# facebookresearch/PoseDiffusion

Measured on AMD Instinct MI355X. Metric: sequences/sec (20-frame, GGS on), higher is better.
Workload: dtype f32 (GGS, attention, LayerNorm, DDPM update, every accumulation); the encoder GEMMs multiply fp16 hi + lo operand pairs (22 bits, static power-of-two scales) with fp32 accumulation -- `exact_mode` is the same pipe with them on the exact-fp32 matrix instruction

## Files before the change

include/pd_engine.h:

```cpp
#ifndef PD_ENGINE_H
#define PD_ENGINE_H

#include <stdint.h>

#ifdef __cplusplus
extern "C" {
#endif

#define PD_OK 0
#define PD_ERR_INVALID_ARG (-1)
#define PD_ERR_UNSUPPORTED (-2)
#define PD_ERR_HIP (-3)
#define PD_ERR_STATE (-4)

#define PD_MAX_LAYERS 16
#define PD_POSE_DIM 9

typedef struct pd_engine pd_engine;

typedef struct pd_layer_weights {
    const float *norm1_w, *norm1_b;
    const float *in_proj_w, *in_proj_b;
    const float *out_proj_w, *out_proj_b;
    const float *norm2_w, *norm2_b;
// ... 88 lines not shown
                                 const double *kp2, const int64_t *i12, int n_frames, int height, int width,
                                 const pd_match_hints *hints, void *stream);


int pd_ggs_guide(pd_engine *eng, float *model_mean, int B, int N, int t, const pd_ggs_cfg *cfg,
                 float *stats_out, void *stream);

int pd_ggs_stage_iters(const pd_ggs_cfg *cfg, int *iters_out5);

int pd_ggs_optimize(pd_engine *eng, float *model_mean, int B, int N, int update_R, int update_T,
                    int update_FL, const pd_ggs_cfg *cfg, float *stats_out, float *trace_out,
                    void *stream);

int pd_ggs_loss_grad(pd_engine *eng, const float *x, int B, int N, int update_R, int update_T,
                     int update_FL, const pd_ggs_cfg *cfg, float *loss_out, float *grad_out,
                     void *stream);


#define PD_OPT_DENOISER_SPLIT 2
#define PD_OPT_DENOISER_FUSED_ATTN 5
#define PD_OPT_DENOISER_LONG_ATTN 6
#define PD_OPT_GGS_MAX_FRAMES 7
#define PD_OPT_GGS_LONG_PAIR_ITEMS 8
int pd_engine_set_option(pd_engine *eng, int option, int value);
#define PD_OPT_WEIGHTS_NON_FINITE 4
int pd_engine_get_option(pd_engine *eng, int option, int *value_out);

int pd_sample(pd_engine *eng, const float *z, const float *noise, int B, int N, int cond_start_step,
              const pd_ggs_cfg *ggs, float *pose_out, float *process_out, float *stats_out,
              int use_graph, void *stream);

#define PD_PHASE_ALL 0
#define PD_PHASE_UNGUIDED 1
#define PD_PHASE_GUIDED 2
int pd_sample_phase(pd_engine *eng, const float *z, const float *noise, int B, int N, int cond_start_step,
                    const pd_ggs_cfg *ggs, int phase, float *pose_out, float *process_out, float *stats_out,
                    int use_graph, void *stream);

int pd_pose_to_camera(pd_engine *eng, const float *enc, int n_cameras, float *R_out, float *T_out,
                      float *focal_out, void *stream);
int pd_pose_to_camera_ex(pd_engine *eng, const float *enc, int n_cameras, float *R_out, float *T_out,
                         float *focal_out, float log_focal_length_bias, float min_focal_length, float max_focal_length,
                         void *stream);

int pd_camera_to_pose(const float *R, const float *T, const float *focal, int n, float log_focal_length_bias,
                      float min_focal_length, float max_focal_length, float *enc_out, void *stream);
// ... 58 lines not shown
```

posediffusion_amd/_lib.py:

```python
from __future__ import annotations

import ctypes as C
import os
import subprocess

_HERE = os.path.dirname(os.path.abspath(__file__))
LIB_PATH = os.environ.get("PD_ENGINE_LIB") or os.path.join(_HERE, "lib", "libpd_engine.so")
CSRC_DIR = os.path.join(_HERE, "csrc")
HEADER_PATH = os.path.normpath(os.path.join(_HERE, "..", "include", "pd_engine.h"))

PD_MAX_LAYERS = 16

c_float_p = C.POINTER(C.c_float)


class pd_layer_weights(C.Structure):
    _fields_ = [(n, C.c_void_p) for n in (
        "norm1_w", "norm1_b", "in_proj_w", "in_proj_b", "out_proj_w", "out_proj_b",
        "norm2_w", "norm2_b", "linear1_w", "linear1_b", "linear2_w", "linear2_b")]


class pd_weights(C.Structure):
    _fields_ = (
        [(n, C.c_int32) for n in ("d_model", "nhead", "dim_ff", "num_layers", "z_dim", "n_harmonic",
# ... 27 lines not shown
class pd_vit_weights(C.Structure):
    _fields_ = ([(n, C.c_int32) for n in ("dim", "depth", "num_heads", "mlp_hidden", "patch_size", "pos_grid", "reserved0", "reserved1")]
                + [(n, C.c_void_p) for n in ("patch_w", "patch_b", "cls_token", "pos_embed", "norm_w", "norm_b")]
                + [("layers", pd_vit_layer_weights * 16)])


PD_GGS_CFG_FORCE_ONE_HOP = 1
PD_GGS_CFG_NO_LDS_STAGING = 2
PD_GGS_CFG_WAVES8 = 4
PD_WEIGHTS_PRED_X0 = 1
PD_WEIGHTS_POST_NORM = 2
PD_WEIGHTS_NO_PIVOT = 4
PD_WEIGHTS_GENERIC = 8
PD_GGS_CFG_LANE_ITEMS = 8
PD_GGS_CFG_NO_LANE_ITEMS = 16
PD_GGS_CFG_XCHG_SPREAD = 32
PD_GGS_CFG_LONG_FRAMES = 64
PD_OPT_DENOISER_SPLIT = 2
PD_OPT_WEIGHTS_NON_FINITE = 4
PD_OPT_DENOISER_FUSED_ATTN = 5
PD_OPT_DENOISER_LONG_ATTN = 6
PD_OPT_GGS_MAX_FRAMES = 7
PD_OPT_GGS_LONG_PAIR_ITEMS = 8
PD_DROP_ATTN, PD_DROP_RESID1, PD_DROP_FF, PD_DROP_RESID2, PD_DROP_ALL = 1, 2, 4, 8, 15
PD_TR_OPT_MAX_FRAMES, PD_TR_OPT_LONG_ATTN = 1, 2
PD_MATCH_HINT_ONE_ORDER = 1 << 30


class pd_ggs_cfg(C.Structure):
    _fields_ = [("alpha", C.c_float), ("learning_rate", C.c_float), ("iter_num", C.c_int32),
                ("sampson_max", C.c_float), ("min_matches", C.c_int32), ("momentum", C.c_float),
                ("wgs_per_seq", C.c_int32), ("reserved", C.c_int32)]


class pd_match_hints(C.Structure):
    _fields_ = [("max_pairs", C.c_int32), ("max_matches_per_pair", C.c_int32)]


_vp, _i, _i64 = C.c_void_p, C.c_int, C.c_int64
SIGNATURES = {
    "pd_engine_create": (_i, [C.POINTER(pd_weights), _i, _i, C.POINTER(_vp)]),
    "pd_engine_destroy": (None, [_vp]),
    "pd_last_error": (C.c_char_p, []),
    "pd_version": (C.c_char_p, []),
    "pd_denoise_step": (_i, [_vp, _vp, _vp, _i, _i, _i, _vp, _vp]),
    "pd_engine_set_q_tables": (_i, [_vp, _vp, _vp]),
# ... 96 lines not shown
```

posediffusion_amd/csrc/pd_engine.hip:

```cpp
#include "pd_internal.h"

#include <algorithm>

#include <math.h>
#include <stdarg.h>
#include <string.h>

static thread_local char g_err[1024] = "";

void pd_set_error(const char *fmt, ...) {
    va_list ap;
    va_start(ap, fmt);
    vsnprintf(g_err, sizeof(g_err), fmt, ap);
    va_end(ap);
}

extern "C" const char *pd_last_error(void) { return g_err; }
extern "C" const char *pd_version(void) { return "pd_engine 0.1 gfx950"; }

__global__ void pd_finish_kernel(const float *__restrict__ mean, const float *__restrict__ noise, float sigma, int n,
                                 float *__restrict__ out, const int *__restrict__ nf, int n_frames) {
    const int i = blockIdx.x * blockDim.x + threadIdx.x;
    if (i >= n) return;
    if (nf) {
// ... 693 lines not shown
            unsigned long long *fresh = nullptr;
            if (hipMalloc((void **)&fresh, sizeof(unsigned long long) * 2 * granules * eng->max_B) != hipSuccess) {
                (void)hipGetLastError();
                pd_set_error("pd_engine_set_option: PD_OPT_GGS_MAX_FRAMES = %d: hipMalloc of %zu B for the exchange region failed; the limit stays %d",
                             value, sizeof(unsigned long long) * 2 * granules * eng->max_B, eng->ggs_max_frames);
                return PD_ERR_HIP;
            }
            (void)hipFree(eng->d_xchg);
            eng->d_xchg = fresh;
            eng->xchg_granules = granules;
        }
        for (auto &g : eng->graphs) (void)hipGraphExecDestroy(g.second);
        eng->graphs.clear();
        eng->ggs_max_frames = value;
        break;
    }
    case PD_OPT_GGS_LONG_PAIR_ITEMS:
        if (value < 0 || value > 1) {
            pd_set_error("pd_engine_set_option: PD_OPT_GGS_LONG_PAIR_ITEMS takes 0 or 1 (got %d)", value);
            return PD_ERR_INVALID_ARG;
        }
        eng->ggs_long_pair_items = value;
        break;
    case 3:
        if (value == 0) break;
        pd_set_error("pd_engine_set_option: option 3 (the persistent small-batch denoiser launch of round 3) is no longer built: it measured "
                     "2.4 x slower than the multi-launch path (profiles/round3_small_persistent.txt; source parked under tools/parked/)");
        return PD_ERR_UNSUPPORTED;
    default:
        pd_set_error("pd_engine_set_option: unknown option %d", option);
        return PD_ERR_INVALID_ARG;
    }
    return PD_OK;
}

extern "C" int pd_engine_get_option(pd_engine *eng, int option, int *value_out) {
    if (!eng || !value_out) {
        pd_set_error("pd_engine_get_option: NULL argument");
        return PD_ERR_INVALID_ARG;
    }
    switch (option) {
    case PD_OPT_DENOISER_SPLIT: *value_out = eng->den_split; break;
    case PD_OPT_DENOISER_FUSED_ATTN: *value_out = eng->den_fused_attn; break;
    case PD_OPT_DENOISER_LONG_ATTN: *value_out = eng->den_long_attn; break;
    case PD_OPT_GGS_MAX_FRAMES: *value_out = eng->ggs_max_frames; break;
    case PD_OPT_GGS_LONG_PAIR_ITEMS: *value_out = eng->ggs_long_pair_items; break;
    case PD_OPT_WEIGHTS_NON_FINITE: *value_out = pd_denoiser_weights_non_finite(eng) ? 1 : 0; break;
    default:
        pd_set_error("pd_engine_get_option: unknown option %d", option);
        return PD_ERR_INVALID_ARG;
    }
    return PD_OK;
}

extern "C" int pd_time_kernel(pd_engine *eng, int what, int B, int N, const pd_ggs_cfg *cfg, int reps, float *ms_out,
                              void *stream) {
    if (!eng || !ms_out || reps <= 0 || B <= 0 || B > eng->max_B || N <= 0 || N > eng->max_N) {
        pd_set_error("pd_time_kernel: invalid arguments");
        return PD_ERR_INVALID_ARG;
    }
    if (what != 0) {
        PD_TRY(check_cfg(cfg, "pd_time_kernel"));
        PD_TRY(pd_ggs_frames_unsupported(eng, N, "pd_time_kernel"));
    }
    hipStream_t s = (hipStream_t)stream;
    struct CountsOff {
        pd_engine *e;
        int B;
        explicit CountsOff(pd_engine *e_) : e(e_), B(e_->nf_B) { e->nf_B = 0; }
// ... 112 lines not shown
```

posediffusion_amd/csrc/pd_ggs.hip:

```cpp
#include "pd_internal.h"

#include <algorithm>
#include <math.h>
#include <stdlib.h>
#include <string.h>

#pragma clang fp contract(on)

#ifndef PD_GGS_PROF12
#define PD_GGS_PROF12 0
#endif
#ifndef PD_GGS_ABLATE
#define PD_GGS_ABLATE 0
#endif

#ifndef PD_GGS_MIN_WAVES_PER_SIMD
#define PD_GGS_MIN_WAVES_PER_SIMD 2
#endif

#include "pd_ggs_lds.h"
#include "pd_ggs_dev.h"
#include "pd_ggs_sampson.h"
#include "pd_ggs_kernels.h"
#include "pd_ggs_lane.inc"
// ... 46 lines not shown
    max_items = 0;
    for (int b = 0; b < B; ++b) {
        const PdSeqDesc &d = eng->seqs[b].desc;
        if (d.M <= 0 || !eng->seqs[b].blob) {
            pd_set_error("pd_ggs: sequence slot %d has no matches (call pd_ggs_set_matches)", b);
            return PD_ERR_STATE;
        }
        const int n_b = nf_dev ? eng->nf_host[b] : N;
        if (d.n_frames != n_b) {
            if (nf_dev) pd_set_error("pd_ggs: slot %d matches were uploaded for %d frames, its frame count (pd_engine_set_frame_counts) is %d", b, d.n_frames, n_b);
            else pd_set_error("pd_ggs: slot %d matches were uploaded for %d frames, called with N=%d", b, d.n_frames, N);
            return PD_ERR_INVALID_ARG;
        }
        max_items = std::max(max_items, d.n_items);
    }
    return PD_OK;
}

static bool plan_lane(const pd_engine *eng, int B, int N, const pd_ggs_cfg *cfg, int device_cus, PdGgsPlan *out) {
    if ((cfg->reserved & PD_GGS_CFG_NO_LANE_ITEMS) ||
        !((cfg->reserved & PD_GGS_CFG_LANE_ITEMS) || (cfg->wgs_per_seq == 0 && device_cus / B <= 1)))
        return false;
    bool ok = N <= PD_GGS_FAST_FRAMES;
    int pairs = 0, steps = 0, deg = 0;
    for (int b = 0; b < B && ok; ++b) {
        const PdSeqDesc &d = eng->seqs[b].desc;
        ok = d.n_litems > 0 && d.n_pchunks == 1;
        pairs = std::max(pairs, d.n_pairs);
        steps = std::max(steps, d.l_max_steps);
        deg = std::max(deg, eng->seqs[b].max_deg);
    }
    if (!ok) return false;
    const int pinc_rows = std::max(2 * std::min(PD_LANE_MAX_ITEMS, std::max(pairs, 1)), N * (((deg + 3) & ~3) + 1));
    const size_t lds = lane_lds_bytes(pinc_rows, PD_LANE_SLOTS);
    if (lds > 160 * 1024) return false;
    out->lane = 1;
    out->lane_rl = std::max(0, std::min(PD_LANE_RL, steps - PD_LANE_RV));
    out->k = 1;
    out->waves = PD_LANE_WAVES;
    out->pinc_rows = pinc_rows;
    out->lds = (int)lds;
    out->max_items = PD_LANE_MAX_ITEMS;
    return true;
}

static int plan_wave_items(const pd_engine *eng, int B, int N, const pd_ggs_cfg *cfg, int device_cus, int k, int max_items, PdGgsPlan *out) {
    if (k > 1 && (size_t)max_items * PD_XCHG_LINE > eng->xchg_granules) k = 1;
    bool two_hop = k > 1 && !(cfg->reserved & PD_GGS_CFG_FORCE_ONE_HOP);
    for (int b = 0; b < B && two_hop; ++b) {
        const PdSeqDesc &d = eng->seqs[b].desc;
        two_hop = d.n_pchunks > 1 && d.single_item_pairs;
    }
    int max_pairs = 0, max_len = 0;
    for (int b = 0; b < B; ++b) {
        max_pairs = std::max(max_pairs, eng->seqs[b].desc.n_pairs);
        max_len = std::max(max_len, eng->seqs[b].max_item_len);
    }
    int pinc_one_hop = std::min(PD_GGS_PINC_ROWS, 2 * std::min(PD_GGS_THREADS, std::max(max_pairs, 1)));
    int pinc_fast = 0;
    if (N <= PD_GGS_FAST_FRAMES) {
        int deg = 0;
        bool one_chunk = true;
        for (int b = 0; b < B; ++b) {
            deg = std::max(deg, eng->seqs[b].max_deg);
// ... 187 lines not shown
    if (!eng || !x || !cfg || n_stages <= 0 || n_stages > PD_GGS_MAX_STAGES) {
        pd_set_error("pd_ggs: invalid arguments (B=%d N=%d stages=%d)", B, N, n_stages);
        return PD_ERR_INVALID_ARG;
    }
    if (trace && eng->nf_B) {
        pd_set_error("pd_ggs_optimize: trace_out must be NULL while frame counts per sequence are set (pd_engine_set_frame_counts)");
        return PD_ERR_INVALID_ARG;
    }
    PdGgsPlan plan;
    PD_TRY(pd_ggs_plan(eng, B, N, cfg, &plan));
    PD_TRY(pd_wait_uploads(eng, s));
    const PdGgsParams P = launch_params(eng, x, B, N, stages, n_stages, cfg, eval_only, stats, trace, trace_iters, loss_out, grad_out, plan);
    if (plan.k > 1) {
        const size_t n_zero = 2 * eng->xchg_granules * B;
        hipLaunchKernelGGL(pd_ggs_zero_kernel, dim3(256), dim3(256), 0, s, eng->d_xchg, n_zero);
    }
    const size_t lds = (size_t)plan.lds;
    const int B_map = plan.xchg_local ? ((B + 7) & ~7) : B;
    if (plan.long_frames == 2)
        hipLaunchKernelGGL(pd_ggs_longm_kernel, dim3(B * plan.k), dim3(PD_GGS_THREADS), lds, s, P, B, plan.n_slots, plan.pinc_rows / 2);
    else if (plan.long_frames)
        hipLaunchKernelGGL(pd_ggs_long_kernel, dim3(B * plan.k), dim3(PD_GGS_THREADS), lds, s, P, B, plan.n_slots, plan.pinc_rows / 2);
    else if (plan.lane)
        hipLaunchKernelGGL(pd_ggs_lane_kernel<PD_LANE_RV>, dim3(B), dim3(PD_LANE_THREADS), lds, s, P, plan.pinc_rows);
    else if (plan.two_hop)
        hipLaunchKernelGGL(pd_ggs2_kernel, dim3(B * plan.k), dim3(PD_GGS_THREADS), lds, s, P, B, plan.n_slots);
    else {
        const PdGgsKernel kern = ggs_variant(plan.stage_p, plan.n_slots == PD_GGS_WAVES, plan.waves);
        if (!kern) {
            pd_set_error("pd_ggs: no pd_ggs_kernel variant for stage_p=%d n_slots=%d waves=%d", plan.stage_p, plan.n_slots, plan.waves);
            return PD_ERR_STATE;
        }
        hipLaunchKernelGGL(kern, dim3(B_map * plan.k), dim3(plan.waves * 64), lds, s, P, B_map, plan.n_slots, plan.pinc_rows, plan.max_items);
    }
    PD_HIP_CHECK(hipGetLastError());
    return pd_mark_use(eng, s);
}
```

posediffusion_amd/csrc/pd_ggs_kernels.h:

```cpp
#pragma once
#include "pd_ggs_sampson.h"

template <int STAGE_P, bool RESIDENT, int NW = PD_GGS_WAVES>
__global__ __launch_bounds__(NW * 64, NW > PD_GGS_WAVES ? 3 : PD_GGS_MIN_WAVES_PER_SIMD) void pd_ggs_kernel(PdGgsParams P, int B, int n_slots, int pinc_rows, int items_cap) {
    constexpr int NT = NW * 64;
    constexpr bool SINGLE = NW > PD_GGS_WAVES;
    static_assert(!(RESIDENT && SINGLE) && (NW == PD_GGS_WAVES || STAGE_P > 0), "12 waves: the staged variants only");
    extern __shared__ __attribute__((aligned(16))) float smem[];
    const int tid = threadIdx.x, lane = tid & 63;
    const int wave = tid >> 6;
    const int b = blockIdx.x % B, wg = blockIdx.x / B;
    if (b >= P.n_seqs) return;
    const PdSeqDesc D = P.seqs[b];
    const int N = D.n_frames, k = P.k;
    const int nW = k * PD_GGS_WAVES;
    const int n_items = D.n_items;
    const Lds L = carve(smem, n_slots, pinc_rows, items_cap);
    const bool p3t = tid < PD_GGS_THREADS;
    float *xg = P.x + (size_t)b * P.N * PD_POSE_DIM;
    u64 *xchg = P.xchg ? P.xchg + (size_t)b * 2 * P.xchg_stride : nullptr;

    const bool own = (wave == 0 && lane < N);
    if (wave == 0) {
#pragma unroll
// ... 369 lines not shown
                            float Wr[9];
                            jac_row_x(qn, x, Wr);
                            const float *ps = L.psum + n * 16;
#pragma unroll
                            for (int m = 0; m < 9; ++m) v = __builtin_fmaf(m < 6 ? -ps[m] : ps[m], Wr[m], v);
                        }
                    } else if (x < 7) {
                        if (S.update_T) {
                            const float t = L.psum[n * 16 + 9 + (x - 4)];
                            v = (x - 4 < 2) ? -t : t;
                        }
                    }
                    L.gq[q] = v;
                }
                if (tid < 4) {
                    float v = 0.0f;
                    for (int n = 0; n < N; ++n) v += L.psum[n * 16 + 12 + tid];
                    L.gA[tid] = v;
                }
            }
            __syncthreads();
            PD_PROF(3);

#include "pd_ggs_p4q.inc"
            __syncthreads();
            PD_PROF(4);
            if (prof && lane == 0) L.prof[5] += 1;
            if (L.ctl[0] != 0.0f) break;
        }
        if (wave == 0 && lane == 0 && wg == 0 && P.stats) {
            float *so = P.stats + ((size_t)b * P.n_stages + st) * 4;
            so[0] = L.ctl[5];
            so[1] = (float)stepped;
            so[2] = L.ctl[6];
            so[3] = L.ctl[7];
        }
        if (P.eval_only) break;
    }
    if (prof && lane == 0) {
        for (int i = 0; i < 16; ++i) P.prof[i] = L.prof[i];
    }
    if (own && wg == 0 && !P.eval_only) {
#pragma unroll
        for (int c = 0; c < 9; ++c) xg[lane * 9 + c] = L.xst[lane * PD_XS_STRIDE + c];
    }
    if (STAGE_P > 0) pd_vmcnt<0>();
// ... 735 lines not shown
```

posediffusion_amd/csrc/pd_ggs_lane.inc:

```

#ifndef PD_LANE_RV
#define PD_LANE_RV 14
#endif
#ifndef PD_LANE_PAIRED
#define PD_LANE_PAIRED (PD_LANE_WAVES < 12)
#endif
#ifndef PD_LANE_RING
#define PD_LANE_RING 3
#endif
#ifndef PD_LANE_RL
#define PD_LANE_RL 3
#endif
#define PD_LANE_SLOTS (PD_LANE_RING + PD_LANE_RL)
#ifndef PD_LANE_ZIGZAG
#define PD_LANE_ZIGZAG 0
#endif

typedef float pd_f4v __attribute__((ext_vector_type(4)));
typedef const pd_f4v __attribute__((address_space(1))) *pd_gf4p;
__device__ __forceinline__ float4 pd_nt_load4(pd_gf4p p, unsigned lane) {
    const pd_f4v t = __builtin_nontemporal_load(p + lane);
    return make_float4(t.x, t.y, t.z, t.w);
}
__device__ __forceinline__ float4 pd_g_load4(pd_gf4p p, unsigned lane) {
    const pd_f4v t = p[lane];
    return make_float4(t.x, t.y, t.z, t.w);
}

#define PD_LANE_STEP(MASKED, q0, q1, t)                                                                                              \
    do {                                                                                                                             \
        const float4 a_ = (q0), b_ = (q1);                                                                                           \
        const v2f u1_ = {a_.x, a_.y}, v1_ = {a_.z, a_.w}, u2_ = {b_.x, b_.y}, v2_ = {b_.z, b_.w};                                     \
        if (MASKED) sampson_step2<EXACT>(u1_, v1_, u2_, v2_, 2 * (t) < cnt, 2 * (t) + 1 < cnt, Fp, smax, acc2, mind, nv, vmask);     \
        else sampson_step2<EXACT>(u1_, v1_, u2_, v2_, true, true, Fp, smax, acc2, mind, nv, vmask);                                  \
    } while (0)

// ... 63 lines not shown
                                          unsigned long long vmask, const PdFPairs &Fp, float smax, v2f (&acc2)[PD_ITEM_VALS], float &mind, int &nv) {
    mind = __int_as_float(0x7f800000);
    nv = 0;
#pragma unroll
    for (int c = 0; c < PD_ITEM_VALS; ++c) acc2[c] = (v2f){0.0f, 0.0f};
    const bool full_res = !EXACT && tfull >= RV && T >= RV;
    static_assert(RV % 2 == 0, "register-resident steps are consumed in pairs");
    if (full_res) {
#pragma unroll
        for (int t = 0; t < RV; t += 2) {
            if (PD_LANE_PAIRED) {
                PD_LANE_STEP2(false, rv[2 * t], rv[2 * t + 1], t, rv[2 * t + 2], rv[2 * t + 3], t + 1);
            } else {
                PD_LANE_STEP(false, rv[2 * t], rv[2 * t + 1], t);
                PD_LANE_STEP(false, rv[2 * t + 2], rv[2 * t + 3], t + 1);
            }
        }
    } else {
#pragma unroll
        for (int t = 0; t < RV; ++t)
            if (t < T) PD_LANE_STEP(true, rv[2 * t], rv[2 * t + 1], t);
    }
    int t = RV;
    if constexpr (PD_LANE_RL > 0) {
        const int t_res = min(RV + PD_LANE_RL, T);
        if (PD_LANE_PAIRED) {
            for (; t + 2 <= min(t_res, tfull); t += 2) {
                const float4 *p = R.res + (t - RV) * 128;
                PD_LANE_STEP2(false, p[0], p[64], t, p[128], p[192], t + 1);
            }
        }
        for (; t < t_res; ++t) {
            const float4 *p = R.res + (t - RV) * 128;
            PD_LANE_STEP(true, p[0], p[64], t);
        }
    }
    const bool refill = R.n_s > PD_LANE_RING;
    if (!refill) R.slot = 0;
    const int S0 = t, n = T - t;
    const int d = (PD_LANE_ZIGZAG && refill && !R.fwd) ? -1 : 1;
    if (d < 0) t = T - 1;
    int done = 0;
    if (PD_LANE_PAIRED && n >= 2) {
        const int tf = min(max(tfull, S0), T), np = n >> 1;
        const int nu_up = (tf - S0) >> 1;
        const int nm_dn = min(np, T - 1 >= tf ? ((T - 1 - tf) >> 1) + 1 : 0);
        const int seg0 = d > 0 ? 0 : nm_dn, seg1 = d > 0 ? nu_up : np - nm_dn, seg2 = d > 0 ? np - nu_up : 0;
        for (int k = 0; k < seg0; ++k, t += 2 * d) {
// ... 5 lines not shown
        for (int k = 0; k < seg1; ++k, t += 2 * d) {
            float4 a0, a1, b0, b1;
            lane_ring_take<2 * PD_LANE_RING - 2>(R, lane16, a0, a1, refill);
            lane_ring_take<2 * PD_LANE_RING - 2>(R, lane16, b0, b1, refill);
            PD_LANE_STEP2(false, a0, a1, t, b0, b1, t + d);
        }
        for (int k = 0; k < seg2; ++k, t += 2 * d) {
            float4 a0, a1, b0, b1;
            lane_ring_take<2 * PD_LANE_RING - 2>(R, lane16, a0, a1, refill);
            lane_ring_take<2 * PD_LANE_RING - 2>(R, lane16, b0, b1, refill);
            PD_LANE_STEP2(true, a0, a1, t, b0, b1, t + d);
        }
        done = 2 * np;
    }
    for (; done < n; ++done, t += d) {
        float4 a0, a1;
        lane_ring_take<2 * PD_LANE_RING - 2>(R, lane16, a0, a1, refill);
        PD_LANE_STEP(true, a0, a1, t);
    }
    if (PD_LANE_ZIGZAG && refill) R.fwd ^= 1;
}

template <int RV>
__global__ __launch_bounds__(PD_LANE_THREADS, PD_LANE_WAVES / 4) void pd_ggs_lane_kernel(PdGgsParams P, int pinc_rows) {
    constexpr int NT = PD_LANE_THREADS;
    constexpr int wg = 0;
    extern __shared__ __attribute__((aligned(16))) float smem[];
    const int tid = threadIdx.x, lane = tid & 63;
    const int wave = __builtin_amdgcn_readfirstlane(tid >> 6);
    const int b = blockIdx.x;
    const PdSeqDesc D = P.seqs[b];
    const int N = D.n_frames;
    const Lds L = carve_lane(smem, pinc_rows);
    if (tid == 0) {
        if (P.stamp && b == 0) P.stamp[0] = wall_clock64();
        ((unsigned *)L.psum)[14] = (unsigned)(size_t)P.stamp;
        ((unsigned *)L.psum)[15] = (unsigned)((size_t)P.stamp >> 32);
    }
    float *xg = P.x + (size_t)b * P.N * PD_POSE_DIM;
    const float smax = P.sampson_max;

    const bool own = (wave == 0 && lane < N);
    if (wave == 0) {
#pragma unroll
        for (int c = 0; c < 9; ++c) {
            L.xst[lane * PD_XS_STRIDE + c] = own ? xg[lane * 9 + c] : 0.0f;
            L.mst[lane * PD_XS_STRIDE + c] = 0.0f;
        }
    }
    for (int q = tid; q <= N; q += NT) L.incoff[q] = D.n_pchunks > 0 ? D.pchunk_off[q] : 0;
    if (tid == 0) {
        L.ctl[0] = 0.0f;
        L.ctl[1] = 0.0f;
    }
    if (wave == 0) {
        float xr0[9];
        params_load(L.xst, lane, xr0);
        decode_all(L, xr0, lane, N, D);
    }
    const bool has_item = tid < D.n_litems;
    const int4 li = has_item ? D.litems[tid] : make_int4(0, 0, 0, 0);
    const int pi = li.x & 0xff, pj = li.x >> 8, cnt = li.y;
    int wbase = 0, T = 0;
    if (wave < D.n_lwaves) {
        const int2 lw = D.lwave[wave];
        wbase = __builtin_amdgcn_readfirstlane(lw.x);
        T = __builtin_amdgcn_readfirstlane(lw.y);
    }
    const unsigned long long vmask = __builtin_amdgcn_ballot_w64(has_item);
    int tf = has_item ? (cnt >> 1) : 0x7fffffff;
#pragma unroll
    for (int d = 32; d >= 1; d >>= 1) tf = min(tf, __shfl_xor(tf, d, 64));
    const int tfull = vmask ? __builtin_amdgcn_readfirstlane(tf) : 0;
    pd_gf4p sw = (pd_gf4p)D.lstream + wbase;
    float4 rv[2 * RV];
#pragma unroll
    for (int t = 0; t < RV; ++t) {
        const int tt = max(min(t, T - 1), 0);
        rv[2 * t] = pd_g_load4(sw + (size_t)tt * 128, lane);
        rv[2 * t + 1] = pd_g_load4(sw + (size_t)tt * 128 + 64, lane);
    }
    LaneRing R;
    R.n_s = max(T - RV - PD_LANE_RL, 0);
    R.src = (const float4 *)D.lstream + wbase + (size_t)(RV + PD_LANE_RL) * 128;
    float *wave_lds = L.stage + wave * (PD_LANE_SLOTS * 512);
    R.res = (const float4 *)wave_lds + lane;
    R.lds0 = __builtin_amdgcn_readfirstlane((unsigned)(size_t)(wave_lds + PD_LANE_RL * 512));
    R.rd = (const float4 *)(wave_lds + PD_LANE_RL * 512) + lane;
    R.slot = 0;
    const unsigned lane16 = (unsigned)lane * 16u;
    {
        if constexpr (PD_LANE_RL > 0) {
            const int nr = max(min(T - RV, PD_LANE_RL), 0);
            for (int u = 0; u < nr; ++u)
                lane_dma_step((const float4 *)D.lstream + wbase + (size_t)(RV + u) * 128, (unsigned)(size_t)(wave_lds + u * 512), lane16);
        }
        const int n0 = min(R.n_s, PD_LANE_RING);
        R.next = 0;
        R.dir = 1;
        R.fwd = 1;
        for (int u = 0; u < n0; ++u) {
            lane_ring_fetch(R, u, u, lane16);
            if (R.n_s > PD_LANE_RING) lane_ring_advance(R);
        }
        if (PD_LANE_RL > 0 || R.n_s <= PD_LANE_RING) pd_vmcnt<0>();
    }
    __syncthreads();

    int cap = 0;
    for (int n = 0; n < N; ++n) cap = max(cap, L.incoff[n + 1] - L.incoff[n]);
    cap = (cap + 3) & ~3;
    const int rstride = cap + 1, n_row_waves = (N * 16 + 63) >> 6, ga_parts = n_row_waves;
    const bool p3a = tid < D.n_pairs;
    int4 my_pair = p3a ? D.ptab[tid] : make_int4(0, 0, 0, 0);
    if (p3a) {
        const int fi = my_pair.x & 0xff, fj = my_pair.x >> 8;
        my_pair.w = (fi * rstride + ((my_pair.w & 0xffff) - L.incoff[fi])) | ((fj * rstride + ((my_pair.w >> 16) - L.incoff[fj])) << 16);
    }
    for (int q = tid; q < N * rstride * 4; q += NT) ((float4 *)L.pinc)[q] = make_float4(0.0f, 0.0f, 0.0f, 0.0f);
    if (wave == PD_LANE_WAVES - 1) jac_all(L, lane, N);
    const int2 my_lp = p3a ? D.lptab[tid] : make_int2(0, 0);
    int trace_row = 0;
    const float inv_M = 1.0f / (float)D.M;
    const bool prof = P.prof != nullptr && b == 0 && wave == (P.prof_wave & 7);
    long long pt0 = 0, pt1 = 0, pt2 = 0, pt3 = 0, pit = 0, pc = 0;
#define PD_LPROF(acc) do { if (prof) { const long long n_ = __builtin_amdgcn_s_memtime(); acc += n_ - pc; pc = n_; } } while (0)
    for (int st = 0; st < P.n_stages; ++st) {
        const PdGgsStage S = P.stages[st];
// ... 23 lines not shown
                }
                v2f acc2[PD_ITEM_VALS];
                float mind;
                int nv;
                lane_pass<false, RV>(rv, R, lane16, T, tfull, cnt, vmask, Fp, smax, acc2, mind, nv);
                const float band = smax * (PD_SAMPSON_BAND_ULPS * 1.1920929e-7f);
                if ((__builtin_amdgcn_ballot_w64(mind <= band) & vmask) != 0ull)
                    lane_pass<true, RV>(rv, R, lane16, T, tfull, cnt, vmask, Fp, smax, acc2, mind, nv);
                if (has_item) {
#pragma unroll
                    for (int c = 0; c < 9; ++c) {
                        const float h = acc2[c].x + acc2[c].y;
                        L.item[tid * PD_LANE_ITEM_VALS + c] = h + h;
                    }
                    L.item[tid * PD_LANE_ITEM_VALS + 9] = acc2[9].x + acc2[9].y;
                }
                if (lane == 0) L.psum[wave] = (float)nv;
            }
            if (wave == PD_LANE_WAVES - 1 && S.update_R) jac_all(L, lane, N);
            PD_LPROF(pt0);
            __syncthreads();
            PD_LPROF(pt1);

            if (p3a) {
                const int4 mp = my_pair;
                const int pi = mp.x & 0xff, pj = mp.x >> 8;
                float G[9];
#pragma unroll
                for (int c = 0; c < 9; ++c) G[c] = 0.0f;
                for (int u = 0; u < my_lp.y; ++u)
#pragma unroll
                    for (int c = 0; c < 9; ++c) G[c] += L.item[(my_lp.x + u) * PD_LANE_ITEM_VALS + c];
#include "pd_ggs_pairbwd.inc"
            }
            if (wave == PD_LANE_WAVES - 1) {
                float s_sum = 0.0f;
                for (int q2 = lane; q2 < D.n_litems; q2 += 64) s_sum += L.item[q2 * PD_LANE_ITEM_VALS + 9];
                s_sum = wave_allsum(s_sum);
                const float s_cnt = wave_allsum(lane < PD_LANE_WAVES ? L.psum[lane] : 0.0f);
                if (lane == 0) {
                    L.cam[6] = s_sum;
                    L.cam[7] = s_cnt;
                    L.ctl[2] = s_sum + smax * ((float)D.M - s_cnt);
                }
            }
            __syncthreads();
            {
                int tid_b = tid;
                asm volatile("" : "+v"(tid_b));
                const int fb_n = tid_b >> 4, fb_c = tid_b & 15;
                const float fb_sign = (fb_c < 9) ? (fb_c < 6 ? -1.0f : 1.0f) : ((fb_c < 11) ? -1.0f : 1.0f);
#include "pd_ggs_p3b.inc"
            }
            __syncthreads();
            PD_LPROF(pt2);

#include "pd_ggs_p4q.inc"
            __syncthreads();
            PD_LPROF(pt3);
            pit += 1;
            if (L.ctl[0] != 0.0f) break;
        }
        if (wave == 0 && lane == 0 && P.stats) {
            float *so = P.stats + ((size_t)b * P.n_stages + st) * 4;
            so[0] = L.ctl[5];
            so[1] = (float)stepped;
            so[2] = L.ctl[6];
            so[3] = L.ctl[7];
        }
        if (P.eval_only) break;
    }
    if (prof && lane == 0) {
        P.prof[0] = 0;
        P.prof[1] = pt0;
        P.prof[2] = pt1;
        P.prof[3] = pt2;
        P.prof[4] = pt3;
        P.prof[5] = pit;
    }
// ... 14 lines not shown
```

posediffusion_amd/csrc/pd_ggs_lds.h:

```cpp
#pragma once
#include "pd_internal.h"

#define PD_F_STRIDE 12
#define PD_GGS_PSUM_FLOATS (PD_GGS_FAST_FRAMES * 48 > 64 * 16 ? PD_GGS_FAST_FRAMES * 48 : 64 * 16)
#define PD_FR_STRIDE 12
#define PD_XS_STRIDE 12
struct Lds {
    float *Rc;
    float *fl;
    float *cam;
    float *gT;
    float *gR;
    float *gA;
    float *ctl;
    long long *prof;
    float *xst;
    float *mst;
    float *pinc;
    float *psum;
    float *W;
    float *gq;
    int4 *itab;
    int *incoff;
    float *F;
// ... 14 lines not shown
    L.xst = L.ctl + 8 + 32;
    L.mst = L.xst + 64 * PD_XS_STRIDE;
    L.pinc = L.mst + 64 * PD_XS_STRIDE;
    L.psum = L.pinc + pinc_rows * 16;
    L.W = L.psum;
    L.gq = L.gR;
    L.itab = (int4 *)(L.psum + PD_GGS_PSUM_FLOATS);
    L.incoff = (int *)(L.itab + n_slots);
    L.F = (float *)(L.incoff + PD_GGS_MAX_PCHUNKS * 68);
    L.item = L.F + n_slots * PD_F_STRIDE;
    L.stage = base + ((((L.item + n_items_cap * PD_ITEM_VALS) - base) + 255) & ~255);
    return L;
}

static float *pd_ggs_lds_origin() { return (float *)(size_t)(1u << 20); }
static size_t pd_ggs_lds_offset(const void *p) { return (size_t)((const char *)p - (const char *)pd_ggs_lds_origin()); }

static size_t ggs_lds_bytes(int n_slots, int n_items, int pinc_rows, int stage_p, int stage_bufs = PD_GGS_WAVES * 2) {
    const Lds L = carve(pd_ggs_lds_origin(), n_slots, pinc_rows, n_items);
    if (stage_p > 0) return pd_ggs_lds_offset(L.stage) + (size_t)stage_bufs * stage_p * 1024;
    return pd_ggs_lds_offset(L.item + (size_t)n_items * PD_ITEM_VALS);
}

__host__ __device__ __forceinline__ Lds carve_lane(float *base, int pinc_rows) {
    Lds L;
    L.Rc = base;
    L.fl = L.Rc + 48 * PD_FR_STRIDE;
    L.cam = L.fl + 48 * 4;
    L.gT = L.cam + 8;
    L.gR = L.gT + 48 * 3;
    L.gA = L.gR + 48 * 9;
    L.ctl = L.gA + 48 * 4;
    L.xst = L.ctl + 8;
    L.mst = L.xst + 64 * PD_XS_STRIDE;
    L.psum = L.mst + 64 * PD_XS_STRIDE;
    L.W = L.psum + 16;
    L.gq = L.gR;
    L.pinc = L.W + PD_GGS_FAST_FRAMES * 48;
    L.incoff = (int *)(L.pinc + pinc_rows * 16);
    L.item = (float *)(L.incoff + 68);
    L.itab = nullptr;
    L.F = nullptr;
    L.stage = base + ((((L.item + PD_LANE_MAX_ITEMS * PD_LANE_ITEM_VALS) - base) + 255) & ~255);
    return L;
}
static size_t lane_lds_bytes(int pinc_rows, int wave_slots) {
    return pd_ggs_lds_offset(carve_lane(pd_ggs_lds_origin(), pinc_rows).stage) + (size_t)wave_slots * PD_LANE_WAVES * 2048;
}
static bool lane_pinc_aligned() { return pd_ggs_lds_offset(carve_lane(pd_ggs_lds_origin(), 0).pinc) % 16 == 0; }

#define PD_GGS_LONG_FRAMES 256
#define PD_GGS_LONG_INCOFF 260
#define PD_GGS_LONG_FRAME_ROWS 512
#define PD_GGS_LONG_TOT_ROWS 256
#define PD_GGS_LONG_RED 32
struct LdsLong : Lds {
    float *red;
    float *tot_rows;
    float *frame_rows;
    float *own_rows;
    int *grow;
    float *end;
};
__host__ __device__ __forceinline__ LdsLong carve_long(float *base, int n_slots, int n_batch) {
    constexpr int NF = PD_GGS_LONG_FRAMES;
    LdsLong L;
    L.Rc = base;
    L.fl = L.Rc + NF * PD_FR_STRIDE;
    L.cam = L.fl + NF * 4;
    L.gT = L.cam + 8;
    L.gR = L.gT + NF * 3;
    L.gA = L.gR + NF * 9;
// ... 29 lines not shown
```

posediffusion_amd/csrc/pd_ggs_p4q.inc:

```
            if (wave == 0 && (PD_GGS_ABLATE & 8)) {
                if (lane == 0) L.ctl[0] = 0.0f;
            } else if (wave == 0) {
                float xr[9], mom[9];
                params_load(L.xst, lane, xr);
                params_load(L.mst, lane, mom);
                const float s_sum = L.cam[6], s_cnt = L.cam[7], s_cl = L.ctl[2];
                const float last_print = s_cl * inv_M;
                if (lane == 0) {
                    L.ctl[5] = last_print;
                    L.ctl[6] = s_cnt;
                }
                const bool done = (!P.eval_only) && P.min_matches > 0 && (s_cnt < (float)P.min_matches * (float)N);
                if (!done) {
                    const float inv_cnt = pd_rcp(s_cnt);
                    const float loss = s_sum * inv_cnt;
                    if (lane == 0) L.ctl[7] = loss;
                    float g[9];
#pragma unroll
                    for (int c = 0; c < 9; ++c) g[c] = 0.0f;
                    if (lane < N) {
                        const float4 gq4 = *(const float4 *)&L.gq[lane * 8], gt4 = *(const float4 *)&L.gq[lane * 8 + 4];
                        g[0] = gt4.x * inv_cnt;
                        g[1] = gt4.y * inv_cnt;
                        g[2] = gt4.z * inv_cnt;
// ... 48 lines not shown
                        const float coef = fminf(max_norm * pd_rcp(gnorm + 1e-6f), 1.0f);
#pragma unroll
                        for (int c = 0; c < 9; ++c) {
                            const float gc = g[c] * coef;
                            mom[c] = (stepped == 0) ? gc : P.momentum * mom[c] + gc;
                            xr[c] = xr[c] - P.lr * mom[c];
                        }
                        ++stepped;
                        if (P.trace && wg == 0 && trace_row < P.trace_iters) {
                            float *tr = P.trace + ((size_t)b * P.trace_iters + trace_row) * (N * 9 + 3);
                            if (lane < N) {
                                int lo_ = lane;
                                asm volatile("" : "+v"(lo_));
#pragma unroll
                                for (int c = 0; c < 9; ++c) tr[lo_ * 9 + c] = xr[c];
                            }
                            if (lane == 0) {
                                tr[N * 9 + 0] = loss;
                                tr[N * 9 + 1] = s_cnt;
                                tr[N * 9 + 2] = gnorm;
                            }
                        }
                        ++trace_row;
                        params_store(L.xst, lane, xr);
                        params_store(L.mst, lane, mom);
                        decode_all(L, xr, lane, N, D, S.update_R != 0, S.update_T != 0, S.update_FL != 0);
                    }
                }
                if (lane == 0) L.ctl[0] = (done || P.eval_only) ? 1.0f : 0.0f;
            }
```

posediffusion_amd/csrc/pd_internal.h:

```cpp
#pragma once

#include <hip/hip_runtime.h>
#include <stdint.h>
#include <stdio.h>
#include <string>
#include <vector>

#include "../../include/pd_engine.h"

#define PD_WAVE 64
#define PD_MAX_FRAMES 64
#define PD_GGS_LONG_MAX_FRAMES 256
#define PD_MAX_DENOISER_FRAMES 256
#define PD_GGS_THREADS 512
#define PD_GGS_WAVES (PD_GGS_THREADS / PD_WAVE)
#define PD_GGS_PINC_ROWS (2 * PD_GGS_THREADS)
#define PD_GGS_MAX_PCHUNKS 8
#define PD_GGS_MAX_STAGES 5
#define PD_ITEM_MAX_MATCHES 512
#define PD_ITEM_VALS 12
#ifndef PD_LANE_WAVES
#define PD_LANE_WAVES 8
#endif
#define PD_LANE_THREADS (PD_LANE_WAVES * PD_WAVE)
// ... 182 lines not shown
struct PdGenericDen;

struct pd_engine {
    int device = 0;
    int num_cus = 0;
    int max_B = 0, max_N = 0;
    int d_model = 0, nhead = 0, dim_ff = 0, num_layers = 0, z_dim = 0, timesteps = 0;
    PdDenoiserDev *den = nullptr;
    PdGenericDen *gden = nullptr;
    std::vector<float> c_recip, c_recipm1, coef1, coef2, logvar;
    int pred_x0 = 0;
    float *d_c_recip = nullptr, *d_c_recipm1 = nullptr;
    float *d_q_a = nullptr, *d_q_b = nullptr;
    int *d_t_row = nullptr;
    float *d_xt = nullptr;
    int nf_B = 0;
    std::vector<int> nf_host;
    int *d_nf = nullptr;
    std::vector<PdSeqHost> seqs;
    PdSeqDesc *d_seqs = nullptr;
    unsigned long long *d_xchg = nullptr;
    size_t xchg_granules = 0;
    int ggs_max_frames = PD_MAX_FRAMES;
    int ggs_long_pair_items = 0;
    unsigned int *d_err = nullptr;
    int ggs_prof_on = 0;
    int den_fused_attn = 1;
    int den_long_attn = 0;
    int den_split = 0;
    int gemm_wide_min_tiles = 200;
    float *d_stats_scratch = nullptr;
    unsigned long long *d_stamps = nullptr;
    int stamp_slot = 0;
    float *d_z = nullptr, *d_noise = nullptr, *d_process = nullptr, *d_mean = nullptr, *d_stats = nullptr;
    struct GraphKey {
        int B, N, cond_start, has_ggs, phase, den_split;
        pd_ggs_cfg cfg;
        PdGgsPlan plan;
    };
    std::vector<std::pair<GraphKey, hipGraphExec_t>> graphs;
    hipStream_t own_stream = nullptr;
    struct StreamEvent {
        hipStream_t stream;
        hipEvent_t event;
    };
    std::vector<StreamEvent> uses, uploads;
// ... 52 lines not shown
```

Before: 1068.

## Size lane-kernel LDS tables by frame count and grow resident stream slots

The GGS lane kernel's LDS layout is now carved from the actual frame count rather than fixed 48/64-frame tables. Optionally the per-item reduction buffer can alias the pairwise-increment region, with the item reads moved ahead of a barrier and the increments zeroed afterwards. The LDS this frees goes to more resident stream-step slots per wave (up to 6 instead of a fixed 3), so fewer loss-stream steps have to be re-fetched through the ring each iteration. Two new engine options cap the resident count and force item sharing; the cost is an extra barrier when sharing and more host-side planning logic.

Result: no change. 1072 (median of 6 runs) (+0.4%).

```diff
diff --git a/include/pd_engine.h b/include/pd_engine.h
--- a/include/pd_engine.h
+++ b/include/pd_engine.h
@@ -134,6 +134,8 @@
 #define PD_OPT_DENOISER_LONG_ATTN 6
 #define PD_OPT_GGS_MAX_FRAMES 7
 #define PD_OPT_GGS_LONG_PAIR_ITEMS 8
+#define PD_OPT_GGS_LANE_RL_CAP 9
+#define PD_OPT_GGS_LANE_SHARE_ITEMS 10
 int pd_engine_set_option(pd_engine *eng, int option, int value);
 #define PD_OPT_WEIGHTS_NON_FINITE 4
 int pd_engine_get_option(pd_engine *eng, int option, int *value_out);
diff --git a/posediffusion_amd/_lib.py b/posediffusion_amd/_lib.py
--- a/posediffusion_amd/_lib.py
+++ b/posediffusion_amd/_lib.py
@@ -73,6 +73,8 @@
 PD_OPT_DENOISER_LONG_ATTN = 6
 PD_OPT_GGS_MAX_FRAMES = 7
 PD_OPT_GGS_LONG_PAIR_ITEMS = 8
+PD_OPT_GGS_LANE_RL_CAP = 9
+PD_OPT_GGS_LANE_SHARE_ITEMS = 10
 PD_DROP_ATTN, PD_DROP_RESID1, PD_DROP_FF, PD_DROP_RESID2, PD_DROP_ALL = 1, 2, 4, 8, 15
 PD_TR_OPT_MAX_FRAMES, PD_TR_OPT_LONG_ATTN = 1, 2
 PD_MATCH_HINT_ONE_ORDER = 1 << 30
diff --git a/posediffusion_amd/csrc/pd_engine.hip b/posediffusion_amd/csrc/pd_engine.hip
--- a/posediffusion_amd/csrc/pd_engine.hip
+++ b/posediffusion_amd/csrc/pd_engine.hip
@@ -739,6 +739,20 @@
         }
         eng->ggs_long_pair_items = value;
         break;
+    case PD_OPT_GGS_LANE_RL_CAP:
+        if (value < -1) {
+            pd_set_error("pd_engine_set_option: PD_OPT_GGS_LANE_RL_CAP takes -1 (uncapped) or a step count >= 0 (got %d)", value);
+            return PD_ERR_INVALID_ARG;
+        }
+        eng->ggs_lane_rl_cap = value;
+        break;
+    case PD_OPT_GGS_LANE_SHARE_ITEMS:
+        if (value < -1 || value > 1) {
+            pd_set_error("pd_engine_set_option: PD_OPT_GGS_LANE_SHARE_ITEMS takes -1 (where the launch fills the chip), 0 or 1 (got %d)", value);
+            return PD_ERR_INVALID_ARG;
+        }
+        eng->ggs_lane_share_items = value;
+        break;
     case 3:
         if (value == 0) break;
         pd_set_error("pd_engine_set_option: option 3 (the persistent small-batch denoiser launch of round 3) is no longer built: it measured "
@@ -762,6 +776,8 @@
     case PD_OPT_DENOISER_LONG_ATTN: *value_out = eng->den_long_attn; break;
     case PD_OPT_GGS_MAX_FRAMES: *value_out = eng->ggs_max_frames; break;
     case PD_OPT_GGS_LONG_PAIR_ITEMS: *value_out = eng->ggs_long_pair_items; break;
+    case PD_OPT_GGS_LANE_RL_CAP: *value_out = eng->ggs_lane_rl_cap; break;
+    case PD_OPT_GGS_LANE_SHARE_ITEMS: *value_out = eng->ggs_lane_share_items; break;
     case PD_OPT_WEIGHTS_NON_FINITE: *value_out = pd_denoiser_weights_non_finite(eng) ? 1 : 0; break;
     default:
         pd_set_error("pd_engine_get_option: unknown option %d", option);
diff --git a/posediffusion_amd/csrc/pd_ggs.hip b/posediffusion_amd/csrc/pd_ggs.hip
--- a/posediffusion_amd/csrc/pd_ggs.hip
+++ b/posediffusion_amd/csrc/pd_ggs.hip
@@ -92,24 +92,34 @@
         !((cfg->reserved & PD_GGS_CFG_LANE_ITEMS) || (cfg->wgs_per_seq == 0 && device_cus / B <= 1)))
         return false;
     bool ok = N <= PD_GGS_FAST_FRAMES;
-    int pairs = 0, steps = 0, deg = 0;
+    int pairs = 0, steps = 0, deg = 0, items = 0, frames = 0;
     for (int b = 0; b < B && ok; ++b) {
         const PdSeqDesc &d = eng->seqs[b].desc;
         ok = d.n_litems > 0 && d.n_pchunks == 1;
         pairs = std::max(pairs, d.n_pairs);
         steps = std::max(steps, d.l_max_steps);
         deg = std::max(deg, eng->seqs[b].max_deg);
+        items = std::max(items, d.n_litems);
+        frames = std::max(frames, d.n_frames);
     }
     if (!ok) return false;
     const int pinc_rows = std::max(2 * std::min(PD_LANE_MAX_ITEMS, std::max(pairs, 1)), N * (((deg + 3) & ~3) + 1));
-    const size_t lds = lane_lds_bytes(pinc_rows, PD_LANE_SLOTS);
-    if (lds > 160 * 1024) return false;
+    if (lane_lds_bytes_v5(pinc_rows) > 160 * 1024) return false;
+    const int n_items = std::min(items, PD_LANE_MAX_ITEMS);
+    const bool share = eng->ggs_lane_share_items >= 0 ? eng->ggs_lane_share_items != 0 : device_cus / B <= 1;
+    const int rows = share ? lane_region_rows(pinc_rows, n_items) : pinc_rows, own_items = share ? 0 : n_items;
+    int rl = std::min(lane_wave_slots(rows, frames, own_items) - PD_LANE_RING, PD_LANE_RL_MAX);
+    if (rl < 0) return false;
+    if (eng->ggs_lane_rl_cap >= 0) rl = std::min(rl, eng->ggs_lane_rl_cap);
+    rl = std::max(0, std::min(rl, steps - PD_LANE_RV));
     out->lane = 1;
-    out->lane_rl = std::max(0, std::min(PD_LANE_RL, steps - PD_LANE_RV));
+    out->lane_rl = rl;
     out->k = 1;
     out->waves = PD_LANE_WAVES;
-    out->pinc_rows = pinc_rows;
-    out->lds = (int)lds;
+    out->pinc_rows = rows;
+    out->n_slots = frames;
+    out->stage_p = own_items;
+    out->lds = (int)lane_lds_bytes(rows, frames, own_items, PD_LANE_RING + rl);
     out->max_items = PD_LANE_MAX_ITEMS;
     return true;
 }
@@ -343,7 +353,7 @@
     else if (plan.long_frames)
         hipLaunchKernelGGL(pd_ggs_long_kernel, dim3(B * plan.k), dim3(PD_GGS_THREADS), lds, s, P, B, plan.n_slots, plan.pinc_rows / 2);
     else if (plan.lane)
-        hipLaunchKernelGGL(pd_ggs_lane_kernel<PD_LANE_RV>, dim3(B), dim3(PD_LANE_THREADS), lds, s, P, plan.pinc_rows);
+        hipLaunchKernelGGL(pd_ggs_lane_kernel<PD_LANE_RV>, dim3(B), dim3(PD_LANE_THREADS), lds, s, P, plan.pinc_rows, plan.n_slots, plan.lane_rl, plan.stage_p);
     else if (plan.two_hop)
         hipLaunchKernelGGL(pd_ggs2_kernel, dim3(B * plan.k), dim3(PD_GGS_THREADS), lds, s, P, B, plan.n_slots);
     else {
diff --git a/posediffusion_amd/csrc/pd_ggs_kernels.h b/posediffusion_amd/csrc/pd_ggs_kernels.h
--- a/posediffusion_amd/csrc/pd_ggs_kernels.h
+++ b/posediffusion_amd/csrc/pd_ggs_kernels.h
@@ -415,6 +415,7 @@
             __syncthreads();
             PD_PROF(3);
 
+            constexpr bool p4_row_ok = true;
 #include "pd_ggs_p4q.inc"
             __syncthreads();
             PD_PROF(4);
diff --git a/posediffusion_amd/csrc/pd_ggs_lane.inc b/posediffusion_amd/csrc/pd_ggs_lane.inc
--- a/posediffusion_amd/csrc/pd_ggs_lane.inc
+++ b/posediffusion_amd/csrc/pd_ggs_lane.inc
@@ -8,10 +8,9 @@
 #ifndef PD_LANE_RING
 #define PD_LANE_RING 3
 #endif
-#ifndef PD_LANE_RL
-#define PD_LANE_RL 3
+#ifndef PD_LANE_RL_MAX
+#define PD_LANE_RL_MAX 6
 #endif
-#define PD_LANE_SLOTS (PD_LANE_RING + PD_LANE_RL)
 #ifndef PD_LANE_ZIGZAG
 #define PD_LANE_ZIGZAG 0
 #endif
@@ -121,8 +120,8 @@
             if (t < T) PD_LANE_STEP(true, rv[2 * t], rv[2 * t + 1], t);
     }
     int t = RV;
-    if constexpr (PD_LANE_RL > 0) {
-        const int t_res = min(RV + PD_LANE_RL, T);
+    {
+        const int t_res = T - R.n_s;
         if (PD_LANE_PAIRED) {
             for (; t + 2 <= min(t_res, tfull); t += 2) {
                 const float4 *p = R.res + (t - RV) * 128;
@@ -174,7 +173,7 @@
 }
 
 template <int RV>
-__global__ __launch_bounds__(PD_LANE_THREADS, PD_LANE_WAVES / 4) void pd_ggs_lane_kernel(PdGgsParams P, int pinc_rows) {
+__global__ __launch_bounds__(PD_LANE_THREADS, PD_LANE_WAVES / 4) void pd_ggs_lane_kernel(PdGgsParams P, int pinc_rows, int tab_frames, int rl, int own_items) {
     constexpr int NT = PD_LANE_THREADS;
     constexpr int wg = 0;
     extern __shared__ __attribute__((aligned(16))) float smem[];
@@ -183,7 +182,7 @@
     const int b = blockIdx.x;
     const PdSeqDesc D = P.seqs[b];
     const int N = D.n_frames;
-    const Lds L = carve_lane(smem, pinc_rows);
+    const Lds L = carve_lane(smem, pinc_rows, tab_frames, own_items);
     if (tid == 0) {
         if (P.stamp && b == 0) P.stamp[0] = wall_clock64();
         ((unsigned *)L.psum)[14] = (unsigned)(size_t)P.stamp;
@@ -193,7 +192,7 @@
     const float smax = P.sampson_max;
 
     const bool own = (wave == 0 && lane < N);
-    if (wave == 0) {
+    if (wave == 0 && lane < ((tab_frames + 3) & ~3)) {
 #pragma unroll
         for (int c = 0; c < 9; ++c) {
             L.xst[lane * PD_XS_STRIDE + c] = own ? xg[lane * 9 + c] : 0.0f;
@@ -233,17 +232,17 @@
         rv[2 * t + 1] = pd_g_load4(sw + (size_t)tt * 128 + 64, lane);
     }
     LaneRing R;
-    R.n_s = max(T - RV - PD_LANE_RL, 0);
-    R.src = (const float4 *)D.lstream + wbase + (size_t)(RV + PD_LANE_RL) * 128;
-    float *wave_lds = L.stage + wave * (PD_LANE_SLOTS * 512);
+    R.n_s = max(T - RV - rl, 0);
+    R.src = (const float4 *)D.lstream + wbase + (size_t)(RV + rl) * 128;
+    float *wave_lds = L.stage + wave * ((PD_LANE_RING + rl) * 512);
     R.res = (const float4 *)wave_lds + lane;
-    R.lds0 = __builtin_amdgcn_readfirstlane((unsigned)(size_t)(wave_lds + PD_LANE_RL * 512));
-    R.rd = (const float4 *)(wave_lds + PD_LANE_RL * 512) + lane;
+    R.lds0 = __builtin_amdgcn_readfirstlane((unsigned)(size_t)(wave_lds + rl * 512));
+    R.rd = (const float4 *)(wave_lds + rl * 512) + lane;
     R.slot = 0;
     const unsigned lane16 = (unsigned)lane * 16u;
     {
-        if constexpr (PD_LANE_RL > 0) {
-            const int nr = max(min(T - RV, PD_LANE_RL), 0);
+        {
+            const int nr = max(min(T - RV, rl), 0);
             for (int u = 0; u < nr; ++u)
                 lane_dma_step((const float4 *)D.lstream + wbase + (size_t)(RV + u) * 128, (unsigned)(size_t)(wave_lds + u * 512), lane16);
         }
@@ -255,7 +254,7 @@
             lane_ring_fetch(R, u, u, lane16);
             if (R.n_s > PD_LANE_RING) lane_ring_advance(R);
         }
-        if (PD_LANE_RL > 0 || R.n_s <= PD_LANE_RING) pd_vmcnt<0>();
+        if (rl > 0 || R.n_s <= PD_LANE_RING) pd_vmcnt<0>();
     }
     __syncthreads();
 
@@ -325,20 +324,40 @@
             __syncthreads();
             PD_LPROF(pt1);
 
+            float G[9];
+#pragma unroll
+            for (int c = 0; c < 9; ++c) G[c] = 0.0f;
+            if (p3a) {
+                for (int u = 0; u < my_lp.y; ++u)
+#pragma unroll
+                    for (int c = 0; c < 9; ++c) G[c] += L.item[(my_lp.x + u) * PD_LANE_ITEM_VALS + c];
+            }
+            float s_sum = 0.0f;
+            if (wave == PD_LANE_WAVES - 1) {
+                int lane_c = lane;
+                asm volatile("" : "+v"(lane_c));
+                float sv[PD_LANE_MAX_ITEMS / 64];
+#pragma unroll
+                for (int k = 0; k < PD_LANE_MAX_ITEMS / 64; ++k)
+                    sv[k] = L.item[(lane_c + 64 * k) * PD_LANE_ITEM_VALS + 9];
+#pragma unroll
+                for (int k = 0; k < PD_LANE_MAX_ITEMS / 64; ++k)
+                    if (lane_c + 64 * k < D.n_litems) s_sum += sv[k];
+            }
+            if (own_items == 0) {
+                __syncthreads();
+                int tid_z = NT - 1 - tid;
+                asm volatile("" : "+v"(tid_z));
+                const int zf = tid_z >> 4, zc = tid_z & 15;
+                if (zf < N)
+                    for (int e = L.incoff[zf + 1] - L.incoff[zf]; e < cap; ++e) L.pinc[(zf * rstride + e) * 16 + zc] = 0.0f;
+            }
             if (p3a) {
                 const int4 mp = my_pair;
                 const int pi = mp.x & 0xff, pj = mp.x >> 8;
-                float G[9];
-#pragma unroll
-                for (int c = 0; c < 9; ++c) G[c] = 0.0f;
-                for (int u = 0; u < my_lp.y; ++u)
-#pragma unroll
-                    for (int c = 0; c < 9; ++c) G[c] += L.item[(my_lp.x + u) * PD_LANE_ITEM_VALS + c];
 #include "pd_ggs_pairbwd.inc"
             }
             if (wave == PD_LANE_WAVES - 1) {
-                float s_sum = 0.0f;
-                for (int q2 = lane; q2 < D.n_litems; q2 += 64) s_sum += L.item[q2 * PD_LANE_ITEM_VALS + 9];
                 s_sum = wave_allsum(s_sum);
                 const float s_cnt = wave_allsum(lane < PD_LANE_WAVES ? L.psum[lane] : 0.0f);
                 if (lane == 0) {
@@ -358,6 +377,7 @@
             __syncthreads();
             PD_LPROF(pt2);
 
+            const bool p4_row_ok = lane < ((tab_frames + 3) & ~3);
 #include "pd_ggs_p4q.inc"
             __syncthreads();
             PD_LPROF(pt3);
diff --git a/posediffusion_amd/csrc/pd_ggs_lds.h b/posediffusion_amd/csrc/pd_ggs_lds.h
--- a/posediffusion_amd/csrc/pd_ggs_lds.h
+++ b/posediffusion_amd/csrc/pd_ggs_lds.h
@@ -60,32 +60,50 @@
     return pd_ggs_lds_offset(L.item + (size_t)n_items * PD_ITEM_VALS);
 }
 
-__host__ __device__ __forceinline__ Lds carve_lane(float *base, int pinc_rows) {
+__host__ __device__ __forceinline__ Lds carve_lane(float *base, int rows, int n_frames, int own_items) {
+    const int nf = (n_frames + 3) & ~3;
     Lds L;
     L.Rc = base;
-    L.fl = L.Rc + 48 * PD_FR_STRIDE;
-    L.cam = L.fl + 48 * 4;
+    L.fl = L.Rc + nf * PD_FR_STRIDE;
+    L.cam = L.fl + nf * 4;
     L.gT = L.cam + 8;
-    L.gR = L.gT + 48 * 3;
-    L.gA = L.gR + 48 * 9;
-    L.ctl = L.gA + 48 * 4;
+    L.gR = L.gT + nf * 3;
+    L.gA = L.gR + nf * 9;
+    L.ctl = L.gA + nf * 4;
     L.xst = L.ctl + 8;
-    L.mst = L.xst + 64 * PD_XS_STRIDE;
-    L.psum = L.mst + 64 * PD_XS_STRIDE;
+    L.mst = L.xst + nf * PD_XS_STRIDE;
+    L.psum = L.mst + nf * PD_XS_STRIDE;
     L.W = L.psum + 16;
     L.gq = L.gR;
-    L.pinc = L.W + PD_GGS_FAST_FRAMES * 48;
-    L.incoff = (int *)(L.pinc + pinc_rows * 16);
-    L.item = (float *)(L.incoff + 68);
+    L.incoff = (int *)(L.W + nf * 48);
+    L.pinc = (float *)(L.incoff + 68);
+    L.item = own_items > 0 ? L.pinc + rows * 16 : L.pinc;
     L.itab = nullptr;
     L.F = nullptr;
-    L.stage = base + ((((L.item + PD_LANE_MAX_ITEMS * PD_LANE_ITEM_VALS) - base) + 255) & ~255);
+    float *end = own_items > 0 ? L.item + own_items * PD_LANE_ITEM_VALS : L.pinc + rows * 16;
+    L.stage = base + (((end - base) + 255) & ~255);
     return L;
 }
-static size_t lane_lds_bytes(int pinc_rows, int wave_slots) {
-    return pd_ggs_lds_offset(carve_lane(pd_ggs_lds_origin(), pinc_rows).stage) + (size_t)wave_slots * PD_LANE_WAVES * 2048;
+static int lane_region_rows(int pinc_rows, int n_items) {
+    const int item_rows = (n_items * PD_LANE_ITEM_VALS + 15) / 16;
+    return pinc_rows > item_rows ? pinc_rows : item_rows;
 }
-static bool lane_pinc_aligned() { return pd_ggs_lds_offset(carve_lane(pd_ggs_lds_origin(), 0).pinc) % 16 == 0; }
+static size_t lane_lds_bytes(int rows, int n_frames, int own_items, int wave_slots) {
+    return pd_ggs_lds_offset(carve_lane(pd_ggs_lds_origin(), rows, n_frames, own_items).stage) + (size_t)wave_slots * PD_LANE_WAVES * 2048;
+}
+static int lane_wave_slots(int rows, int n_frames, int own_items) {
+    const long long room = 160 * 1024 - (long long)lane_lds_bytes(rows, n_frames, own_items, 0);
+    return room < 0 ? -1 : (int)(room / (PD_LANE_WAVES * 2048));
+}
+static size_t lane_lds_bytes_v5(int pinc_rows) {
+    const size_t tables = 4 * (size_t)(48 * 32 + 16 + 2 * 64 * PD_XS_STRIDE + 16 + PD_GGS_FAST_FRAMES * 48 + pinc_rows * 16 + 68 + PD_LANE_MAX_ITEMS * 10);
+    return ((tables + 1023) & ~(size_t)1023) + (size_t)6 * PD_LANE_WAVES * 2048;
+}
+static bool lane_pinc_aligned() {
+    for (int n = 1; n <= PD_LANE_MAX_FRAMES; ++n)
+        if (pd_ggs_lds_offset(carve_lane(pd_ggs_lds_origin(), 0, n, 0).pinc) % 16 != 0) return false;
+    return true;
+}
 
 #define PD_GGS_LONG_FRAMES 256
 #define PD_GGS_LONG_INCOFF 260
diff --git a/posediffusion_amd/csrc/pd_ggs_p4q.inc b/posediffusion_amd/csrc/pd_ggs_p4q.inc
--- a/posediffusion_amd/csrc/pd_ggs_p4q.inc
+++ b/posediffusion_amd/csrc/pd_ggs_p4q.inc
@@ -94,8 +94,10 @@
                             }
                         }
                         ++trace_row;
-                        params_store(L.xst, lane, xr);
-                        params_store(L.mst, lane, mom);
+                        if (p4_row_ok) {
+                            params_store(L.xst, lane, xr);
+                            params_store(L.mst, lane, mom);
+                        }
                         decode_all(L, xr, lane, N, D, S.update_R != 0, S.update_T != 0, S.update_FL != 0);
                     }
                 }
diff --git a/posediffusion_amd/csrc/pd_internal.h b/posediffusion_amd/csrc/pd_internal.h
--- a/posediffusion_amd/csrc/pd_internal.h
+++ b/posediffusion_amd/csrc/pd_internal.h
@@ -228,6 +228,8 @@
     unsigned long long *d_xchg = nullptr;
     size_t xchg_granules = 0;
     int ggs_max_frames = PD_MAX_FRAMES;
+    int ggs_lane_share_items = -1;
+    int ggs_lane_rl_cap = -1;
     int ggs_long_pair_items = 0;
     unsigned int *d_err = nullptr;
     int ggs_prof_on = 0;
```
